# zhyever/PatchFusion

Hardware: NVIDIA H100
Metric: tiles/s (higher is better)
Workload: dtype bf16

## Files before the change

### patchfusion_b200/csrc/pf_api.cu

```cuda
#include <cuda_bf16.h>
#include <stdarg.h>
#include <stdio.h>
#include <stdlib.h>
#include <string.h>

#include <atomic>
#include <mutex>
#include <unordered_map>
#include <vector>

#include "pf_kernels.h"

namespace pf {

static thread_local char g_err[512] = "";
static std::atomic<long long> g_launches{0};

int set_error(const char* fmt, ...) {
  va_list ap;
  va_start(ap, fmt);
  vsnprintf(g_err, sizeof(g_err), fmt, ap);
  va_end(ap);
  return 1;
}
// ... 26 lines not shown
  }
}
static std::atomic<int> g_opt[6] = {{-1}, {-1}, {-1}, {-1}, {-1}, {-1}};
int option(int which) {
  static const char* names[6] = {"PF_OPT_TMA_EPILOGUE", "PF_OPT_HALO_MULTICAST", "PF_OPT_GEMM_MULTICAST", "PF_OPT_FUSED_RESAMPLE", "PF_OPT_PDL", "PF_OPT_RESIZE_SEPARABLE"};
  static const int defaults[6] = {1, 1, 1, 0, 0, 0};
  if (which < 0 || which > 5) return 0;
  int v = g_opt[which].load(std::memory_order_relaxed);
  if (v < 0) {
    const char* e = getenv(names[which]);
    if (!e && which == PF_OPT_PDL) e = getenv("PF_B200_PDL");
    v = e ? atoi(e) : defaults[which];
    g_opt[which].store(v, std::memory_order_relaxed);
  }
  return v;
}
bool pdl_enabled() {
  return option(PF_OPT_PDL) != 0;
}
int check_launch(const char* what) {
  cudaError_t e = cudaGetLastError();
  if (e != cudaSuccess) return set_error("%s launch: %s", what, cudaGetErrorString(e));
  count_launch(what);
  return 0;
}

typedef CUresult (*EncodeTiledFn)(CUtensorMap*, CUtensorMapDataType, cuuint32_t, void*, const cuuint64_t*,
                                  const cuuint64_t*, const cuuint32_t*, const cuuint32_t*, CUtensorMapInterleave,
                                  CUtensorMapSwizzle, CUtensorMapL2promotion, CUtensorMapFloatOOBfill);

static EncodeTiledFn encode_fn() {
  static EncodeTiledFn fn = nullptr;
  static std::once_flag once;
  std::call_once(once, [] {
    void* p = nullptr;
    cudaDriverEntryPointQueryResult q;
    if (cudaGetDriverEntryPoint("cuTensorMapEncodeTiled", &p, cudaEnableDefault, &q) == cudaSuccess &&
        q == cudaDriverEntryPointSuccess)
      fn = reinterpret_cast<EncodeTiledFn>(p);
  });
  return fn;
}

struct MapKey {
  uint64_t v[12];
  bool operator==(const MapKey& o) const { return memcmp(v, o.v, sizeof(v)) == 0; }
};
struct MapKeyHash {
  size_t operator()(const MapKey& k) const {
    uint64_t h = 1469598103934665603ull;
    for (int i = 0; i < 12; ++i) { h ^= k.v[i]; h *= 1099511628211ull; }
    return static_cast<size_t>(h);
  }
};
static std::unordered_map<MapKey, CUtensorMap, MapKeyHash> g_maps;
static std::mutex g_maps_mu;

static int encode(CUtensorMap* out, const void* ptr, int rank, const uint64_t* dims, const uint64_t* strides_bytes,
                  const uint32_t* box, CUtensorMapDataType dt = CU_TENSOR_MAP_DATA_TYPE_BFLOAT16) {
  MapKey key;
  memset(&key, 0, sizeof(key));
  key.v[0] = reinterpret_cast<uint64_t>(ptr);
  key.v[1] = static_cast<uint64_t>(rank) | (static_cast<uint64_t>(dt) << 8);
  for (int i = 0; i < rank; ++i) {
    key.v[2 + i] = dims[i];
    key.v[6 + i] = (i + 1 < rank ? strides_bytes[i] : 0) ^ (static_cast<uint64_t>(box[i]) << 48);
  }
  {
    std::lock_guard<std::mutex> g(g_maps_mu);
    auto it = g_maps.find(key);
    if (it != g_maps.end()) { *out = it->second; return 0; }
  }
  EncodeTiledFn fn = encode_fn();
  if (!fn) return set_error("cuTensorMapEncodeTiled entry point unavailable (no CUDA driver?)");
  if (reinterpret_cast<uintptr_t>(ptr) & 15) return set_error("tensor map: base pointer not 16-byte aligned");
  cuuint64_t gdim[5];
  cuuint64_t gstr[4];
  cuuint32_t bx[5], es[5];
  for (int i = 0; i < rank; ++i) { gdim[i] = dims[i]; bx[i] = box[i]; es[i] = 1; }
  for (int i = 0; i + 1 < rank; ++i) {
    gstr[i] = strides_bytes[i];
    if (gstr[i] & 15) return set_error("tensor map: stride %d (%llu B) not a multiple of 16", i, (unsigned long long)gstr[i]);
  }
  CUresult r = fn(out, dt, rank, const_cast<void*>(ptr), gdim, gstr, bx, es,
                  CU_TENSOR_MAP_INTERLEAVE_NONE, CU_TENSOR_MAP_SWIZZLE_128B, CU_TENSOR_MAP_L2_PROMOTION_L2_256B,
                  CU_TENSOR_MAP_FLOAT_OOB_FILL_NONE);
  if (r != CUDA_SUCCESS) {
    return set_error("cuTensorMapEncodeTiled failed (%d): rank %d dims %llu %llu %llu %llu box %u %u %u %u", (int)r, rank,
                     (unsigned long long)dims[0], (unsigned long long)(rank > 1 ? dims[1] : 0),
                     (unsigned long long)(rank > 2 ? dims[2] : 0), (unsigned long long)(rank > 3 ? dims[3] : 0), box[0],
                     rank > 1 ? box[1] : 0, rank > 2 ? box[2] : 0, rank > 3 ? box[3] : 0);
  }
  std::lock_guard<std::mutex> g(g_maps_mu);
  if (g_maps.size() > 65536) g_maps.clear();
  g_maps.emplace(key, *out);
  return 0;
}

int tmap_2d_bf16(CUtensorMap* out, const void* ptr, uint64_t cols, uint64_t rows, uint64_t ld, uint32_t box_cols,
                 uint32_t box_rows) {
  uint64_t dims[2] = {cols, rows};
  uint64_t str[1] = {ld * 2};
  uint32_t box[2] = {box_cols, box_rows};
  return encode(out, ptr, 2, dims, str, box);
}
int tmap_2d_f32(CUtensorMap* out, const void* ptr, uint64_t cols, uint64_t rows, uint64_t ld, uint32_t box_cols,
                uint32_t box_rows) {
  uint64_t dims[2] = {cols, rows};
  uint64_t str[1] = {ld * 4};
  uint32_t box[2] = {box_cols, box_rows};
  return encode(out, ptr, 2, dims, str, box, CU_TENSOR_MAP_DATA_TYPE_FLOAT32);
}
int tmap_3d_bf16(CUtensorMap* out, const void* ptr, uint64_t d0, uint64_t d1, uint64_t d2, uint64_t ld1, uint64_t ld2,
                 uint32_t b0, uint32_t b1, uint32_t b2) {
  uint64_t dims[3] = {d0, d1, d2};
  uint64_t str[2] = {ld1 * 2, ld2 * 2};
  uint32_t box[3] = {b0, b1, b2};
  return encode(out, ptr, 3, dims, str, box);
}
int tmap_4d_nhwc_bf16(CUtensorMap* out, const void* ptr, uint64_t C, uint64_t W, uint64_t H, uint64_t N, uint64_t ld,
                      uint32_t box_c, uint32_t box_w, uint32_t box_h) {
  uint64_t dims[4] = {C, W, H, N};
  uint64_t str[3] = {ld * 2, ld * 2 * W, ld * 2 * W * H};
  uint32_t box[4] = {box_c, box_w, box_h, 1};
  return encode(out, ptr, 4, dims, str, box);
}

__global__ void pack_weight_kernel(const float* __restrict__ w, int N, int N_pad, int num_src, int c0, int c1, int c2,
                                   int taps, const float* __restrict__ scale, __nv_bfloat16* __restrict__ dst,
                                   int Ktot) {
  long long idx = blockIdx.x * static_cast<long long>(blockDim.x) + threadIdx.x;
  long long total = static_cast<long long>(N_pad) * Ktot;
  if (idx >= total) return;
  int n = static_cast<int>(idx / Ktot);
  int k = static_cast<int>(idx - static_cast<long long>(n) * Ktot);
  int cs[3] = {c0, c1, c2};
  int ctot = c0 + (num_src > 1 ? c1 : 0) + (num_src > 2 ? c2 : 0);
  float v = 0.0f;
  int cbase = 0, kbase = 0;
  for (int s = 0; s < num_src; ++s) {
    int cp = (cs[s] + 63) / 64 * 64;
    int seg = taps * cp;
    if (k < kbase + seg) {
      int kk = k - kbase;
      int tap = kk / cp, c = kk - tap * cp;
      if (n < N && c < cs[s]) {
        v = w[(static_cast<long long>(n) * ctot + cbase + c) * taps + tap];
        if (scale) v *= scale[n];
      }
      break;
    }
    kbase += seg;
    cbase += cs[s];
  }
  dst[idx] = __float2bfloat16(v);
}

__global__ void pack_convT_kernel(const float* __restrict__ w, int Cin, int Cout, int k, __nv_bfloat16* __restrict__ dst,
                                  int Kp) {
  long long idx = blockIdx.x * static_cast<long long>(blockDim.x) + threadIdx.x;
  int Cp = (Cout + 31) / 32 * 32;
  long long total = static_cast<long long>(k) * k * Cp * Kp;
  if (idx >= total) return;
  int row = static_cast<int>(idx / Kp);
  int ci = static_cast<int>(idx - static_cast<long long>(row) * Kp);
  int tap = row / Cp, co = row - tap * Cp;
  float v = 0.0f;
  if (ci < Cin && co < Cout) v = w[(static_cast<long long>(ci) * Cout + co) * k * k + tap];
// ... 139 lines not shown
  } else if (u->a_mode == 1) {
    int bh = u->bh, bw = u->bw;
    if (bh == 0 || bw == 0) choose_tile(u->H, u->W, &bh, &bw);
    if (bh * bw != 128) return set_error("pf_gemm: bh*bw must be 128");
    d.bh = bh; d.bw = bw;
    d.tiles_y = (u->H + bh - 1) / bh; d.tiles_x = (u->W + bw - 1) / bw;
    d.m_tiles = u->NB * d.tiles_y * d.tiles_x;
    for (int s = 0; s < u->num_src; ++s)
      if (tmap_4d_nhwc_bf16(&tmA[s], u->a_ptr[s], u->a_c[s], u->W, u->H, u->NB, u->a_ld[s], 64, bw, bh)) return 1;
  } else {
    d.m_tiles = (u->M + 127) / 128;
    for (int s = 0; s < u->num_src; ++s)
      if (tmap_2d_bf16(&tmA[s], u->a_ptr[s], u->a_c[s], u->M, u->a_ld[s], 64, 128)) return 1;
  }
  u->bh = d.bh; u->bw = d.bw; u->tiles_y = d.tiles_y; u->tiles_x = d.tiles_x; u->m_tiles = d.m_tiles;
  int bn = u->block_n;
  if (bn == 0) {
    if (halo) {
      bn = n_pad % 192 == 0 ? 192 : (n_pad % 128 == 0 ? 128 : (n_pad % 64 == 0 ? 64 : 32));
    } else if (u->ps > 1 || u->w2) {
      const int span = u->ps > 1 ? (u->ps_cout + 31) / 32 * 32 : n_pad;
      for (int w : kGemmWidths)
        if (span % w == 0) bn = w;
      if (u->w2 && bn != n_pad) return set_error("pf_gemm: fused trailing layer needs the whole row in one N tile (N %d)", u->N);
    } else if (n_pad % 128 == 0) {
      const long long t128 = static_cast<long long>(d.m_tiles) * (n_pad / 128), sms = sm_count();
      const long long waves128 = (t128 + sms - 1) / sms, waves256 = (t128 / 2 + sms - 1) / sms;
      bn = n_pad % 256 == 0 && 2 * waves256 <= waves128 ? 256 : 128;
    } else {
      for (int w : kGemmWidths)
        if (n_pad % w == 0) bn = w;
    }
  }
  d.block_n = bn; d.N = u->N; d.n_tiles = (u->N + bn - 1) / bn;
  u->block_n = bn; u->n_tiles = d.n_tiles;
  if (tmap_2d_bf16(&tmB, u->w_ptr, u->Ktot, static_cast<uint64_t>(d.n_tiles) * bn, u->Ktot, 64, bn)) return 1;
  d.bias = u->bias; d.act = u->act;
  d.res1 = static_cast<const __nv_bfloat16*>(u->res1);
  d.res2 = static_cast<const __nv_bfloat16*>(u->res2);
  d.res_ld = u->res_ld;
  d.gamma = u->gamma;
  d.out = u->out; d.out_f32 = u->out_f32 || u->gamma != nullptr; d.out_ld = u->out_ld; d.out_col0 = u->out_col0;
  d.out2 = static_cast<__nv_bfloat16*>(u->out2); d.out2_ld = u->out2_ld;
  if ((u->out_f32 || u->gamma) && reinterpret_cast<uintptr_t>(u->out) % 32 != 0)
    return set_error("pf_gemm: fp32 outputs must be 32-byte aligned (256-bit epilogue stores)");
  d.wide = ((reinterpret_cast<uintptr_t>(u->out) | reinterpret_cast<uintptr_t>(u->out2) | reinterpret_cast<uintptr_t>(u->res1) |
             reinterpret_cast<uintptr_t>(u->res2)) % 32 == 0) &&
           u->out_col0 % 16 == 0 && (d.out_f32 || u->out_ld % 16 == 0) && (!u->out2 || u->out2_ld % 16 == 0) &&
           (!(u->res1 || u->res2) || u->res_ld % 16 == 0);
  d.ps = u->ps > 1 ? u->ps : 1;
  d.n_logical = u->N;
  if (d.ps > 1) {
    if (u->a_mode != 0) return set_error("pf_gemm: pixel shuffle needs a_mode 0");
    int cpad = (u->ps_cout + 31) / 32 * 32;
    if (cpad % bn != 0) return set_error("pf_gemm: padded ps_cout %d must be a multiple of block_n %d", cpad, bn);
    if (u->N != d.ps * d.ps * cpad) return set_error("pf_gemm: pixel shuffle N %d != k*k*pad32(Cout) %d", u->N, d.ps * d.ps * cpad);
    d.ps_cout_pad = cpad;
    d.n_logical = u->ps_cout;
  }
  d.w2 = u->w2; d.b2 = u->b2; d.n2 = u->n2; d.act2 = u->act2; d.skip_main = u->skip_main;
  d.out3 = u->out3; d.out3_ld = u->out3_ld;
  if (d.w2) {
    if (d.n_tiles != 1) return set_error("pf_gemm: fused trailing layer needs the whole row in one N tile (N %d)", u->N);
    if (d.n2 < 1 || d.n2 > 16 || !d.out3) return set_error("pf_gemm: fused trailing layer n2 %d (1..16), out3 required", d.n2);
    if (u->N % 4) return set_error("pf_gemm: fused trailing layer needs N % 4 == 0");
  }
  d.vt = static_cast<__nv_bfloat16*>(u->vt);
  d.vt_col0 = u->vt_col0; d.vt_seq = u->vt_seq; d.vt_seq_pad = u->vt_seq_pad; d.vt_dim = u->vt_dim;
  if (d.vt && (d.vt_col0 % bn) != 0) return set_error("pf_gemm: vt_col0 must be a multiple of block_n");
  int cl = 1;
  if (d.m_tiles >= 4 && static_cast<long long>(d.m_tiles) * d.n_tiles >= sm_count()) {
    if (halo) cl = option(PF_OPT_HALO_MULTICAST) >= 2 ? 4 : (option(PF_OPT_HALO_MULTICAST) == 1 ? 2 : 1);
    else if (option(PF_OPT_GEMM_MULTICAST) != 0 && u->a_mode == 0 && d.ps == 1 && bn % 16 == 0) cl = 2;
  }
  d.halo_cl = halo ? cl : 1;
  const bool mc = cl > 1;
  CUtensorMap tmBh;
  if (mc && tmap_2d_bf16(&tmBh, u->w_ptr, u->Ktot, static_cast<uint64_t>(d.n_tiles) * bn, u->Ktot, 64, bn / cl)) return 1;
  const bool no_tma_epi = option(PF_OPT_TMA_EPILOGUE) == 0;
  CUtensorMap tmOut;
  d.tma_out = 0;
  const uint64_t ocols = static_cast<uint64_t>(u->out_col0) + u->N;
  const bool ends16 = ocols % (d.out_f32 ? 4 : 8) == 0;
  if (!no_tma_epi && !halo && d.ps == 1 && !d.w2 && !d.res1 && !d.res2 && !d.out2 && ends16) {
    if (!d.out_f32 && bn % 64 == 0 && reinterpret_cast<uintptr_t>(u->out) % 16 == 0) {
      if (u->a_mode == 0) {
        if (tmap_2d_bf16(&tmOut, u->out, ocols, u->M, u->out_ld, 64, 16)) return 1;
      } else {
        const uint32_t bwx = d.bw < 16 ? d.bw : 16;
        if (tmap_4d_nhwc_bf16(&tmOut, u->out, ocols, u->W, u->H, u->NB, u->out_ld, 64, bwx, 16 / bwx)) return 1;
      }
      d.tma_out = 1;
    } else if (d.out_f32 && u->a_mode == 0 && u->out_ld % 4 == 0 && reinterpret_cast<uintptr_t>(u->out) % 16 == 0) {
      if (tmap_2d_f32(&tmOut, u->out, ocols, u->M, u->out_ld, 32, 16)) return 1;
      d.tma_out = 2;
    }
  }
  return gemm_launch(d, tmA, tmB, mc ? &tmBh : nullptr, d.tma_out ? &tmOut : nullptr, static_cast<cudaStream_t>(stream));
}

}
```

### patchfusion_b200/csrc/pf_gemm.cu

```cuda
#include "pf_common.cuh"
#include "pf_kernels.h"

namespace pf {

constexpr int kBlockM = 128;
constexpr int kBlockK = 64;
constexpr int kATileBytes = kBlockM * kBlockK * 2;
constexpr int kEpiWarps = 8;
constexpr int kGemmThreads = (kEpiWarps + 1) * 32;
constexpr int kHaloThreads = (kEpiWarps + 3) * 32;
constexpr int kRsWarp0 = kEpiWarps;
constexpr int kMaxSmem = 227 * 1024;
constexpr int kXposeWarp = 16 * 32 * 4;
constexpr int kStageWarp = 2 * kXposeWarp;
constexpr int kBarBytes = 512;

__host__ __device__ constexpr int gemm_stage_bytes(int bn) { return kATileBytes + bn * kBlockK * 2; }
__host__ __device__ constexpr int gemm_stages(int bn) {
  return (kMaxSmem - 1024  - kBarBytes - kEpiWarps * kStageWarp) / gemm_stage_bytes(bn) < 8
             ? (kMaxSmem - 1024 - kBarBytes - kEpiWarps * kStageWarp) / gemm_stage_bytes(bn)
             : 8;
}

struct GemmKernelParams {
// ... 254 lines not shown
__device__ __forceinline__ void epilogue_row(const GemmDesc& d, const float (&acc)[S], float* buf, int lane,
                                             const TileCoord& c, int ocol0, long long orow, bool row_ok,
                                             float (&y2)[kMaxTail]) {
  const int r = lane & 15;
  const float* rowp = buf + r * 32;
  const int sw = xpose16_swz(r) ^ (lane & 16);
  for (int k = 0; 32 * k < 2 * S && c.n0 + 32 * k < d.N; ++k) {
    acc_stage16_k(k, acc, buf, lane);
    __syncwarp();
    epilogue_cols<16, TAILN>(d, rowp, sw, 32 * k + (lane & 16), c, ocol0, orow, row_ok, y2);
    __syncwarp();
  }
}


struct EpiTma {
  const CUtensorMap* tm;
  uint32_t stg;
  uint8_t* stg_ptr;
  int cur;
};

__device__ __forceinline__ int epi_stage_acquire(EpiTma& e, int lane) {
  if (lane == 0) bulk_wait_read1();
  __syncwarp();
  const int off = e.cur * kXposeWarp;
  e.cur ^= 1;
  return off;
}

template <int S, int K = 0>
__device__ __forceinline__ void acc_chunk(int k, const float (&a)[S], float (&v)[16]) {
  if constexpr (K + 1 < S / 16) {
    if (k != K) { acc_chunk<S, K + 1>(k, a, v); return; }
  }
#pragma unroll
  for (int i = 0; i < 16; ++i) v[i] = a[16 * K + i];
}

__device__ __forceinline__ void epi_act(const GemmDesc& d, float (&f)[16]) {
  if (d.act == PF_ACT_RELU) {
#pragma unroll
    for (int j = 0; j < 16; ++j) f[j] = fmaxf(f[j], 0.0f);
  } else if (d.act == PF_ACT_GELU) {
#pragma unroll
    for (int j = 0; j < 16; j += 2) gelu_erf2(f[j], f[j + 1]);
  } else if (d.act == PF_ACT_SOFTPLUS) {
#pragma unroll
    for (int j = 0; j < 16; ++j) f[j] = softplus(f[j]);
  }
}
__device__ __forceinline__ float2 epi_vec2(const float* p, int col, int n_logical) {
  if (col + 1 < n_logical) return __ldg(reinterpret_cast<const float2*>(p + col));
  return make_float2(col < n_logical ? __ldg(p + col) : 0.f, 0.f);
}
__device__ __forceinline__ void epi_frag(const GemmDesc& d, float (&v)[16], int col, bool scale) {
  if (d.bias != nullptr) {
#pragma unroll
    for (int j = 0; j < 4; ++j) {
      const float2 b = epi_vec2(d.bias, col + 8 * j, d.n_logical);
      v[4 * j] += b.x; v[4 * j + 1] += b.y; v[4 * j + 2] += b.x; v[4 * j + 3] += b.y;
    }
  }
  epi_act(d, v);
  if (scale) {
#pragma unroll
    for (int j = 0; j < 4; ++j) {
      const float2 g = epi_vec2(d.gamma, col + 8 * j, d.n_logical);
      v[4 * j] *= g.x; v[4 * j + 1] *= g.y; v[4 * j + 2] *= g.x; v[4 * j + 3] *= g.y;
    }
  }
}

__device__ __forceinline__ void epi_tma_store(const GemmDesc& d, const EpiTma& e, const uint8_t* tile, const TileCoord& c,
                                              int warp, int col) {
  if (d.a_mode == 1) {
    const int r0 = warp * 16;
    const int yy = r0 / d.bw, xx = r0 - yy * d.bw;
    tma_store_4d(e.tm, tile, col, c.x0 + xx, c.y0 + yy, c.img);
  } else {
    tma_store_2d(e.tm, tile, col, c.m0 + warp * 16);
  }
}
template <int S>
__device__ __forceinline__ void epilogue_tile_tma_bf16(const GemmDesc& d, EpiTma& e, const float (&acc)[S],
                                                       const TileCoord& c, int warp, int lane) {
  const int oct = lane >> 4;
  const uint32_t lane_off = (lane & 15) * 128;
  for (int g = 0; 64 * g < 2 * S; ++g) {
    const int lcol = c.n0 + g * 64;
    if (lcol >= d.n_logical) break;
    const int tile = epi_stage_acquire(e, lane);
#pragma unroll
    for (int h = 0; h < 2; ++h) {
      float v[16];
      acc_chunk(2 * g + h, acc, v);
      epi_frag(d, v, lcol + 32 * h + 2 * (lane & 3), false);
#pragma unroll
      for (int p = 0; p < 2; ++p) {
        const int o = 4 * h + 2 * p;
        const uint32_t addr = e.stg + tile + lane_off + (((o + oct) ^ (lane & 7)) << 4);
        stmatrix_x4(addr, pack_bf16(v[8 * p], v[8 * p + 1]), pack_bf16(v[8 * p + 2], v[8 * p + 3]),
                        pack_bf16(v[8 * p + 4], v[8 * p + 5]), pack_bf16(v[8 * p + 6], v[8 * p + 7]));
      }
    }
    fence_proxy_async_smem();
    __syncwarp();
    if (lane == 0) {
      epi_tma_store(d, e, e.stg_ptr + tile, c, warp, d.out_col0 + lcol);
      bulk_commit();
    }
  }
}

template <int S>
__device__ __forceinline__ void epilogue_tile_tma_f32(const GemmDesc& d, EpiTma& e, const float (&acc)[S],
                                                      const TileCoord& c, int warp, int lane) {
  const int r = lane >> 2, q = lane & 3;
  const uint32_t lane_off = r * 128 + (q & 1) * 8;
  for (int ch = 0; 32 * ch < 2 * S; ++ch) {
    const int lcol = c.n0 + ch * 32;
    if (lcol >= d.n_logical) break;
    const int tile = epi_stage_acquire(e, lane);
    float v[16];
    acc_chunk(ch, acc, v);
    epi_frag(d, v, lcol + 2 * q, d.gamma != nullptr);
#pragma unroll
    for (int j = 0; j < 4; ++j) {
      const uint32_t addr = e.stg + tile + lane_off + (((2 * j + (q >> 1)) ^ r) << 4);
      st_shared_v2f(addr, v[4 * j], v[4 * j + 1]);
      st_shared_v2f(addr + 8 * 128, v[4 * j + 2], v[4 * j + 3]);
    }
    fence_proxy_async_smem();
    __syncwarp();
    if (lane == 0) {
      if (d.gamma != nullptr) tma_reduce_add_2d(e.tm, e.stg_ptr + tile, d.out_col0 + lcol, c.m0 + warp * 16);
      else tma_store_2d(e.tm, e.stg_ptr + tile, d.out_col0 + lcol, c.m0 + warp * 16);
      bulk_commit();
    }
  }
}

struct TileIter {
  int first, step, count, rank, n_tiles, cl;
  __device__ __forceinline__ int tile(int i) const {
    if (cl == 1) return i;
    const int nt = i % n_tiles, mp = i / n_tiles;
    return (cl * mp + rank) * n_tiles + nt;
  }
};
__device__ __forceinline__ TileIter make_iter(const GemmDesc& d, int total_tiles, int cl) {
  TileIter it;
  it.cl = cl; it.n_tiles = d.n_tiles;
  if (cl == 1) { it.first = blockIdx.x; it.step = gridDim.x; it.count = total_tiles; it.rank = 0; }
  else { it.first = blockIdx.x / cl; it.step = gridDim.x / cl; it.count = ((d.m_tiles + cl - 1) / cl) * d.n_tiles; it.rank = cluster_ctarank(); }
  return it;
}

__device__ __forceinline__ void tail_store(const GemmDesc& d, long long orow, const float (&y2)[kMaxTail]) {
  float* op = d.out3 + orow * d.out3_ld;
#pragma unroll
  for (int i = 0; i < kMaxTail; ++i) {
    if (i < d.n2) {
      float v2 = y2[i] + (d.b2 != nullptr ? __ldg(d.b2 + i) : 0.f);
      if (d.act2 == PF_ACT_RELU) v2 = fmaxf(v2, 0.f);
      else if (d.act2 == PF_ACT_SOFTPLUS) v2 = softplus(v2);
      else if (d.act2 == PF_ACT_GELU) v2 = gelu_erf(v2);
      op[i] = v2;
    }
  }
}

template <int S>
__device__ __forceinline__ void epilogue_tile(const GemmDesc& d, const TileCoord& c, const float (&acc)[S], int warp,
                                              int lane, float* buf, EpiTma* et) {
  const int r = 16 * warp + (lane & 15);
  bool row_ok;
  long long orow;
  if (d.a_mode == 1) {
    const int yy = r / d.bw, xx = r - yy * d.bw;
    const int y = c.y0 + yy, x = c.x0 + xx;
    row_ok = (y < d.H) && (x < d.W) && (c.img < d.NB);
    orow = (static_cast<long long>(c.img) * d.H + y) * d.W + x;
  } else {
    const int m = c.m0 + r;
    row_ok = m < d.M;
    orow = m;
  }
  int ocol0 = c.n0;
  if (d.ps > 1 && d.a_mode == 0) {
    const int tap = c.n0 / d.ps_cout_pad;
    ocol0 = c.n0 - tap * d.ps_cout_pad;
    const int ky = tap / d.ps, kx = tap - ky * d.ps;
    const int m = c.m0 + r;
    const int img = m / (d.H * d.W);
    const int rem = m - img * d.H * d.W;
    const int y = rem / d.W, x = rem - y * d.W;
    orow = (static_cast<long long>(img) * d.H * d.ps + y * d.ps + ky) * (d.W * d.ps) + x * d.ps + kx;
  }
  if (et != nullptr && d.tma_out != 0 && !(d.vt != nullptr && c.n0 >= d.vt_col0)) {
    if (d.tma_out == 2) {
      epilogue_tile_tma_f32(d, *et, acc, c, warp, lane);
    } else if constexpr (S % 32 == 0) {
      epilogue_tile_tma_bf16(d, *et, acc, c, warp, lane);
    }
    return;
  }
  if (et != nullptr && d.tma_out != 0) {
    if (lane == 0) bulk_wait_read0();
    __syncwarp();
  }
  float y2[kMaxTail];
#pragma unroll
  for (int i = 0; i < kMaxTail; ++i) y2[i] = 0.f;
  if (d.w2 == nullptr) epilogue_row<0>(d, acc, buf, lane, c, ocol0, orow, row_ok, y2);
  else if (d.n2 <= 1) epilogue_row<1>(d, acc, buf, lane, c, ocol0, orow, row_ok, y2);
  else if (d.n2 <= 4) epilogue_row<4>(d, acc, buf, lane, c, ocol0, orow, row_ok, y2);
  else epilogue_row<kMaxTail>(d, acc, buf, lane, c, ocol0, orow, row_ok, y2);
  if (d.w2 != nullptr) {
#pragma unroll
    for (int i = 0; i < kMaxTail; ++i)
      if (i < d.n2) y2[i] += __shfl_xor_sync(0xffffffffu, y2[i], 16);
    if (row_ok && lane < 16) tail_store(d, orow, y2);
  }
}

template <int CL>
__device__ __forceinline__ void release_stage(uint64_t* bar, int lane) {
  __syncwarp();
  if (lane == 0) {
    if (CL > 1) {
#pragma unroll
      for (int r = 0; r < CL; ++r) mbar_arrive_cluster(bar, r);
    } else {
      mbar_arrive(bar);
    }
  }
}

#ifdef PF_GEMM_TIMELINE
constexpr int kTimelineSlots = 8;
__device__ unsigned long long g_gemm_timeline[kTimelineSlots];
struct GemmTimeline {
  long long v[5] = {0, 0, 0, 0, 0};
  __device__ __forceinline__ long long now() const { return clock64(); }
  __device__ __forceinline__ void add(int i, long long t0) { v[i] += clock64() - t0; }
  __device__ __forceinline__ void tile() { v[0] += 1; }
  __device__ __forceinline__ void flush(int slot0, int n) const {
    for (int i = 0; i < n; ++i) atomicAdd(&g_gemm_timeline[slot0 + i], static_cast<unsigned long long>(v[i]));
  }
};
#else
struct GemmTimeline {
  __device__ __forceinline__ long long now() const { return 0; }
  __device__ __forceinline__ void add(int, long long) {}
  __device__ __forceinline__ void tile() {}
  __device__ __forceinline__ void flush(int, int) const {}
};
#endif

template <bool MC, int BN>
__global__ void __launch_bounds__(kGemmThreads, 1) pf_gemm_kernel(const __grid_constant__ GemmKernelParams P) {
  constexpr int CL = MC ? 2 : 1;
  constexpr int stage_bytes = gemm_stage_bytes(BN);
  constexpr int stages = gemm_stages(BN);
  extern __shared__ uint8_t smem_raw[];
  const GemmDesc& d = P.d;
  uint8_t* smem = reinterpret_cast<uint8_t*>((reinterpret_cast<uintptr_t>(smem_raw) + 1023) & ~uintptr_t(1023));
  uint8_t* xpose = smem + stages * stage_bytes;
  uint64_t* full_bar = reinterpret_cast<uint64_t*>(xpose + kEpiWarps * kStageWarp);
  uint64_t* empty_bar = full_bar + stages;

  const int warp = threadIdx.x >> 5;
  const int lane = threadIdx.x & 31;
  pdl_launch_dependents();

  constexpr int kTmaWarp = kEpiWarps;
  if (warp == kTmaWarp && lane == 0) {
    for (int s = 0; s < d.num_src; ++s) prefetch_tmap(&P.tmA[s]);
    prefetch_tmap(&P.tmB);
    for (int s = 0; s < stages; ++s) { mbar_init(&full_bar[s], 1); mbar_init(&empty_bar[s], kEpiWarps * CL); }
    if (d.tma_out) prefetch_tmap(&P.tmOut);
    fence_barrier_init();
  }
  __syncthreads();
  if (MC) cluster_sync_all();
  const TileIter it = make_iter(d, P.total_tiles, CL);
// ... 13 lines not shown
            int dy = d.taps == 9 ? tap / 3 - 1 : 0;
            int dx = d.taps == 9 ? tap % 3 - 1 : 0;
            for (int ch = 0; ch < d.chunks[s]; ++ch, ++kb) {
              const long long tl_w = tl.now();
              mbar_wait(&empty_bar[stage], phase ^ 1);
              tl.add(1, tl_w);
              uint8_t* sa = smem + stage * stage_bytes;
              uint8_t* sb = sa + kATileBytes;
              if (elect_one()) {
                mbar_expect_tx(&full_bar[stage], stage_bytes);
                if (d.a_mode == 0) tma_load_2d(sa, &P.tmA[s], &full_bar[stage], ch * kBlockK, c.m0);
                else tma_load_4d(sa, &P.tmA[s], &full_bar[stage], ch * kBlockK, c.x0 + dx, c.y0 + dy, c.img);
                if (MC) {
                  constexpr int half_rows = BN / 2;
                  tma_load_2d_mc(sb + it.rank * half_rows * 128, &P.tmBh, &full_bar[stage], kb * kBlockK,
                                 c.n0 + it.rank * half_rows, static_cast<uint16_t>(3));
                } else {
                  tma_load_2d(sb, &P.tmB, &full_bar[stage], kb * kBlockK, c.n0);
                }
              }
              if (++stage == stages) { stage = 0; phase ^= 1; }
            }
          }
        }
      }
      tl.add(2, tl_start);
      if (lane == 0) tl.flush(0, 3);
    }
  } else {
    EpiTma et;
    et.tm = &P.tmOut; et.stg_ptr = xpose + warp * kStageWarp; et.stg = smem_u32(et.stg_ptr); et.cur = 0;
    float* buf = reinterpret_cast<float*>(et.stg_ptr);
    const uint32_t a_off = static_cast<uint32_t>((warp >> 2) * 64 * 128);
    float acc[BN / 2];
    int stage = 0; uint32_t phase = 0;
    int rs = 0;
    GemmTimeline tl;
    const long long tl_start = tl.now();
    for (int ti = it.first; ti < it.count; ti += it.step) {
      const TileCoord c = decode_tile(d, it.tile(ti));
      tl.tile();
      const long long tl_main = tl.now();
      uint32_t accum = 0;
      for (int kb = 0; kb < P.k_steps; ++kb) {
        const long long tl_w = tl.now();
        mbar_wait(&full_bar[stage], phase);
        tl.add(1, tl_w);
        const uint32_t sa = smem_u32(smem + stage * stage_bytes);
        const uint64_t adesc = wgmma_desc_k128(sa + a_off);
        const uint64_t bdesc = wgmma_desc_k128(sa + kATileBytes);
        wgmma_fence();
#pragma unroll
        for (int k = 0; k < kBlockK / 16; ++k) Wgmma<BN>::ss(acc, adesc + 2 * k, bdesc + 2 * k, accum | k);
        wgmma_commit();
        accum = 1;
        wgmma_wait<1>();
        if (kb > 0) {
          release_stage<CL>(&empty_bar[rs], lane);
          if (++rs == stages) rs = 0;
        }
        if (++stage == stages) { stage = 0; phase ^= 1; }
      }
      wgmma_wait<0>();
      release_stage<CL>(&empty_bar[rs], lane);
      if (++rs == stages) rs = 0;
      tl.add(2, tl_main);
      const long long tl_epi = tl.now();
      epilogue_tile(d, c, acc, warp, lane, buf, &et);
      __syncwarp();
      tl.add(3, tl_epi);
    }
    if (lane == 0) bulk_wait0();
    tl.add(4, tl_start);
    if (lane == 0 && (warp & 3) == 0) tl.flush(3, 5);
  }
  __syncthreads();
  if (MC) cluster_sync_all();
}

constexpr int kHaloW = 10, kHaloH = 18;
constexpr int kHaloBytes = kHaloW * kHaloH * 128;
constexpr int kHaloSlot = 24 * 1024;
constexpr int kHaloSlots = 3;
constexpr int kHaloBBytes = kMaxSmem - 1024  - kBarBytes - kEpiWarps * kXposeWarp - kHaloSlots * kHaloSlot;
__host__ __device__ constexpr int halo_kc(int bn) {
  return 2 * 9 * bn * kBlockK * 2 <= kHaloBBytes ? 9 : (2 * 3 * bn * kBlockK * 2 <= kHaloBBytes ? 3 : 1);
}
__host__ __device__ constexpr int halo_stages(int bn) {
  return kHaloBBytes / (halo_kc(bn) * bn * kBlockK * 2) < 6 ? kHaloBBytes / (halo_kc(bn) * bn * kBlockK * 2) : 6;
}


__device__ __forceinline__ void rs_coord(int dst, int in, float scale, int& lo, int& hi, float& frac) {
  const float src = scale * dst;
  lo = static_cast<int>(src);
  if (lo > in - 1) lo = in - 1;
  hi = lo + (lo < in - 1 ? 1 : 0);
  frac = src - lo;
}
__device__ __forceinline__ void halo_fill_bilinear(uint32_t slot, const GemmDesc& d, int s, int ch, const TileCoord& c, int lane) {
  const int ih = d.rs_h[s], iw = d.rs_w[s], ld = d.rs_ld[s];
  const __nv_bfloat16* src = d.rs_ptr[s] + static_cast<size_t>(c.img) * ih * iw * ld + ch * kBlockK;
  const int cvalid = d.k_true[s] - ch * kBlockK;
  const float sy = d.rs_sy[s], sx = d.rs_sx[s];
  const int j = lane & 7;
  const bool jok = j * 8 < cvalid && c.img < d.NB;
#pragma unroll 5
  for (int p = lane >> 3; p < kHaloW * kHaloH; p += 4) {
    const int hy = p / kHaloW, hx = p - hy * kHaloW;
    const int Y = c.y0 - 1 + hy, X = c.x0 - 1 + hx;
    uint32_t o0 = 0, o1 = 0, o2 = 0, o3 = 0;
    if (jok && Y >= 0 && Y < d.H && X >= 0 && X < d.W) {
      int y0, y1, x0, x1; float fy, fx;
      rs_coord(Y, ih, sy, y0, y1, fy);
      rs_coord(X, iw, sx, x0, x1, fx);
      const __nv_bfloat16* r0 = src + static_cast<size_t>(y0) * iw * ld + j * 8;
      const __nv_bfloat16* r1 = src + static_cast<size_t>(y1) * iw * ld + j * 8;
      const uint4 ua = __ldg(reinterpret_cast<const uint4*>(r0 + static_cast<size_t>(x0) * ld));
      const uint4 ub = __ldg(reinterpret_cast<const uint4*>(r0 + static_cast<size_t>(x1) * ld));
      const uint4 uc = __ldg(reinterpret_cast<const uint4*>(r1 + static_cast<size_t>(x0) * ld));
      const uint4 ud = __ldg(reinterpret_cast<const uint4*>(r1 + static_cast<size_t>(x1) * ld));
      const float w00 = (1.f - fy) * (1.f - fx), w01 = (1.f - fy) * fx, w10 = fy * (1.f - fx), w11 = fy * fx;
      const uint64_t p00 = pack2f(w00, w00), p01 = pack2f(w01, w01), p10 = pack2f(w10, w10), p11 = pack2f(w11, w11);
      const uint32_t wa[4] = {ua.x, ua.y, ua.z, ua.w}, wb[4] = {ub.x, ub.y, ub.z, ub.w};
      const uint32_t wc[4] = {uc.x, uc.y, uc.z, uc.w}, wd[4] = {ud.x, ud.y, ud.z, ud.w};
      uint32_t ow[4];
#pragma unroll
      for (int k = 0; k < 4; ++k) {
        uint64_t r = mul2(p00, pack2(wa[k] << 16, wa[k] & 0xffff0000u));
        r = fma2(p01, pack2(wb[k] << 16, wb[k] & 0xffff0000u), r);
        r = fma2(p10, pack2(wc[k] << 16, wc[k] & 0xffff0000u), r);
        r = fma2(p11, pack2(wd[k] << 16, wd[k] & 0xffff0000u), r);
        float lo, hi;
        unpack2f(r, lo, hi);
        ow[k] = pack_bf16(lo, hi);
      }
      o0 = ow[0]; o1 = ow[1]; o2 = ow[2]; o3 = ow[3];
    }
    st_shared_v4(slot + p * 128 + ((j ^ (p & 7)) << 4), o0, o1, o2, o3);
  }
}

__device__ __forceinline__ void halo_a_frags(uint32_t ra, int lane, uint32_t (&fa)[4][4]) {
  const uint32_t sw = (ra >> 7) & 7;
#pragma unroll
  for (int k = 0; k < kBlockK / 16; ++k) ldmatrix_x4(ra + (((2 * k + (lane >> 4)) ^ sw) << 4), fa[k]);
}

template <int CL, int BN>
__global__ void __launch_bounds__(kHaloThreads, 1) pf_conv3_halo_kernel(const __grid_constant__ GemmKernelParams P) {
  constexpr bool MC = CL > 1;
  constexpr uint16_t kMask = static_cast<uint16_t>((1u << CL) - 1);
  constexpr int kc = halo_kc(BN);
  constexpr int b_tile_bytes = BN * kBlockK * 2;
  constexpr int b_stage_bytes = kc * b_tile_bytes;
  constexpr int stages = halo_stages(BN);
  extern __shared__ uint8_t smem_raw[];
  const GemmDesc& d = P.d;
  uint8_t* smem = reinterpret_cast<uint8_t*>((reinterpret_cast<uintptr_t>(smem_raw) + 1023) & ~uintptr_t(1023));
  uint8_t* smem_b = smem + kHaloSlots * kHaloSlot;
  uint8_t* xpose = smem_b + stages * b_stage_bytes;
  uint64_t* bars = reinterpret_cast<uint64_t*>(xpose + kEpiWarps * kXposeWarp);
  uint64_t* a_full = bars;
  uint64_t* a_empty = a_full + kHaloSlots;
  uint64_t* b_full = a_empty + kHaloSlots;
  uint64_t* b_empty = b_full + stages;

  const int warp = threadIdx.x >> 5;
  const int lane = threadIdx.x & 31;
  pdl_launch_dependents();
  constexpr int kTmaWarp = kRsWarp0 + 2;
  if (warp == kTmaWarp && lane == 0) {
    for (int s = 0; s < d.num_src; ++s) if (d.rs_h[s] == 0) prefetch_tmap(&P.tmA[s]);
    prefetch_tmap(&P.tmB);
    for (int s = 0; s < kHaloSlots; ++s) { mbar_init(&a_full[s], 1); mbar_init(&a_empty[s], kEpiWarps); }
    for (int s = 0; s < stages; ++s) { mbar_init(&b_full[s], 1); mbar_init(&b_empty[s], kEpiWarps * CL); }
    fence_barrier_init();
  }
  __syncthreads();
  if (MC) cluster_sync_all();
  const TileIter it = make_iter(d, P.total_tiles, CL);
  pdl_wait();

  if (warp >= kEpiWarps) {
    if (warp == kTmaWarp) {
      int as = 0; uint32_t aph = 0;
      int bs = 0; uint32_t bph = 0;
      for (int ti = it.first; ti < it.count; ti += it.step) {
        TileCoord c = decode_tile(d, it.tile(ti));
        int kbase = 0;
        for (int s = 0; s < d.num_src; ++s) {
          const int nch = d.chunks[s];
          for (int ch = 0; ch < nch; ++ch) {
            if (d.rs_h[s] == 0) {
              mbar_wait(&a_empty[as], aph ^ 1);
              if (elect_one()) {
                mbar_expect_tx(&a_full[as], kHaloBytes);
                tma_load_4d(smem + as * kHaloSlot, &P.tmA[s], &a_full[as], ch * kBlockK, c.x0 - 1, c.y0 - 1, c.img);
              }
            }
            if (++as == kHaloSlots) { as = 0; aph ^= 1; }
            for (int tap0 = 0; tap0 < 9; tap0 += kc) {
              mbar_wait(&b_empty[bs], bph ^ 1);
              if (elect_one()) {
                mbar_expect_tx(&b_full[bs], b_stage_bytes);
                if (MC) {
                  constexpr int part_rows = BN / CL;
                  for (int j = 0; j < kc; ++j)
                    tma_load_2d_mc(smem_b + bs * b_stage_bytes + j * b_tile_bytes + it.rank * part_rows * 128, &P.tmBh,
                                   &b_full[bs], (kbase + (tap0 + j) * nch + ch) * kBlockK, c.n0 + it.rank * part_rows,
                                   kMask);
                } else {
                  for (int j = 0; j < kc; ++j)
                    tma_load_2d(smem_b + bs * b_stage_bytes + j * b_tile_bytes, &P.tmB, &b_full[bs],
                                (kbase + (tap0 + j) * nch + ch) * kBlockK, c.n0);
                }
              }
              if (++bs == stages) { bs = 0; bph ^= 1; }
            }
          }
          kbase += 9 * nch;
        }
      }
    } else if (warp < kRsWarp0 + 2 && d.rs_any) {
      int as = 0; uint32_t aph = 0;
      int turn = 0;
      for (int ti = it.first; ti < it.count; ti += it.step) {
        TileCoord c = decode_tile(d, it.tile(ti));
        for (int s = 0; s < d.num_src; ++s) {
          for (int ch = 0; ch < d.chunks[s]; ++ch) {
            if (d.rs_h[s] != 0) {
              if ((turn & 1) == warp - kRsWarp0) {
                mbar_wait(&a_empty[as], aph ^ 1);
                halo_fill_bilinear(smem_u32(smem + as * kHaloSlot), d, s, ch, c, lane);
                __syncwarp();
                if (lane == 0) mbar_arrive(&a_full[as]);
              }
              ++turn;
            }
            if (++as == kHaloSlots) { as = 0; aph ^= 1; }
          }
        }
      }
    }
  } else {
    float* buf = reinterpret_cast<float*>(xpose + warp * kXposeWarp);
    const int arow = 16 * warp + (lane & 15);
    const uint32_t a_off = static_cast<uint32_t>(((arow >> 3) * kHaloW + (arow & 7)) * 128);
    float acc[BN / 2];
    uint32_t fa[2][4][4];
    int as = 0; uint32_t aph = 0;
    int bs = 0; uint32_t bph = 0;
    int rbs = 0;
    for (int ti = it.first; ti < it.count; ti += it.step) {
      const TileCoord c = decode_tile(d, it.tile(ti));
      uint32_t accum = 0;
      for (int s = 0; s < d.num_src; ++s) {
        for (int ch = 0; ch < d.chunks[s]; ++ch) {
          mbar_wait(&a_full[as], aph);
          const uint32_t a_base = smem_u32(smem + as * kHaloSlot) + a_off;
          uint32_t sb = 0;
#pragma unroll
          for (int tap = 0; tap < 9; ++tap) {
            if (tap % kc == 0) {
              mbar_wait(&b_full[bs], bph);
              sb = smem_u32(smem_b + bs * b_stage_bytes);
              if (++bs == stages) { bs = 0; bph ^= 1; }
            }
            halo_a_frags(a_base + static_cast<uint32_t>(((tap / 3) * kHaloW + tap % 3) * 128), lane, fa[tap & 1]);
            const uint64_t bdesc = wgmma_desc_k128(sb + (tap % kc) * b_tile_bytes);
            wgmma_fence();
#pragma unroll
            for (int k = 0; k < kBlockK / 16; ++k) Wgmma<BN>::rs(acc, fa[tap & 1][k], bdesc + 2 * k, accum | k);
            wgmma_commit();
            accum = 1;
            wgmma_wait<1>();
            if (tap > 0 && tap % kc == 0) {
              release_stage<CL>(&b_empty[rbs], lane);
              if (++rbs == stages) rbs = 0;
            }
          }
          wgmma_wait<0>();
          release_stage<CL>(&b_empty[rbs], lane);
          if (++rbs == stages) rbs = 0;
          release_stage<1>(&a_empty[as], lane);
          if (++as == kHaloSlots) { as = 0; aph ^= 1; }
        }
      }
      epilogue_tile(d, c, acc, warp, lane, buf, nullptr);
      __syncwarp();
    }
  }
  __syncthreads();
  if (MC) cluster_sync_all();
}


static int g_sm_counts[kMaxDevices] = {0};

using KernelFn = void (*)(GemmKernelParams);
template <int CL>
static KernelFn halo_kernel_cl(int bn) {
  switch (bn) {
    case 32: return pf_conv3_halo_kernel<CL, 32>;
    case 64: return pf_conv3_halo_kernel<CL, 64>;
    case 128: return pf_conv3_halo_kernel<CL, 128>;
    case 192: return pf_conv3_halo_kernel<CL, 192>;
    default: return nullptr;
  }
}
static KernelFn halo_kernel(int cl, int bn) {
  return cl == 4 ? halo_kernel_cl<4>(bn) : (cl == 2 ? halo_kernel_cl<2>(bn) : halo_kernel_cl<1>(bn));
}
template <bool MC>
static KernelFn gemm_kernel_mc(int bn) {
  switch (bn) {
    case 32: return pf_gemm_kernel<MC, 32>;
    case 64: return pf_gemm_kernel<MC, 64>;
    case 96: return pf_gemm_kernel<MC, 96>;
    case 128: return pf_gemm_kernel<MC, 128>;
    case 192: return pf_gemm_kernel<MC, 192>;
    case 256: return pf_gemm_kernel<MC, 256>;
    default: return nullptr;
  }
}
static KernelFn gemm_kernel(bool mc, int bn) { return mc ? gemm_kernel_mc<true>(bn) : gemm_kernel_mc<false>(bn); }

int gemm_launch(const GemmDesc& d, const CUtensorMap* tmA, const CUtensorMap& tmB, const CUtensorMap* tmBh,
                const CUtensorMap* tmOut, cudaStream_t stream) {
  static bool attr_done[kMaxDevices] = {false};
  const int dev = current_device();
  if (!attr_done[dev]) {
    cudaError_t e = cudaSuccess;
    for (bool mc : {false, true})
      for (int bn : kGemmWidths)
        if (e == cudaSuccess) e = cudaFuncSetAttribute(gemm_kernel(mc, bn), cudaFuncAttributeMaxDynamicSharedMemorySize, kMaxSmem);
    for (int cl : {1, 2, 4})
      for (int bn : {32, 64, 128, 192})
        if (e == cudaSuccess) e = cudaFuncSetAttribute(halo_kernel(cl, bn), cudaFuncAttributeMaxDynamicSharedMemorySize, kMaxSmem);
    if (e != cudaSuccess) return set_error("cudaFuncSetAttribute(gemm kernels): %s", cudaGetErrorString(e));
    cudaDeviceGetAttribute(&g_sm_counts[dev], cudaDevAttrMultiProcessorCount, dev);
    attr_done[dev] = true;
  }
  const int g_sm_count = g_sm_counts[dev];
  {
    const long long rows = d.a_mode == 1 ? static_cast<long long>(d.NB) * d.H * d.W : d.M;
    int ktrue = 0;
    for (int s = 0; s < d.num_src; ++s) ktrue += d.k_true[s];
    const int n_true = d.ps > 1 ? d.n_logical * d.ps * d.ps : d.N;
    note_work(2.0 * rows * ktrue * d.taps * n_true, "%s rows%lld K%dx%d N%d%s%s%s", d.taps == 9 ? "conv3x3" : (d.a_mode == 1 ? "conv1x1" : (d.ps > 1 ? "convT" : "linear")),
              rows, d.taps, ktrue, n_true, d.act ? (d.act == PF_ACT_GELU ? " gelu" : (d.act == PF_ACT_RELU ? " relu" : " softplus")) : "",
              d.gamma ? " gamma" : (d.vt ? " vt" : ""), d.w2 ? " tail" : "");
  }
  GemmKernelParams P;
  for (int s = 0; s < d.num_src; ++s) P.tmA[s] = tmA[s];
  for (int s = d.num_src; s < 3; ++s) P.tmA[s] = tmA[0];
  P.tmB = tmB;
  P.tmBh = tmBh ? *tmBh : tmB;
  P.tmOut = tmOut ? *tmOut : tmB;
  P.d = d;
  if (d.tma_out && !tmOut) return set_error("gemm: tma_out without an output tensor map");
  int ks = 0;
  for (int s = 0; s < d.num_src; ++s) ks += d.chunks[s] * d.taps;
  P.k_steps = ks;
  P.total_tiles = d.m_tiles * d.n_tiles;
  if (P.total_tiles <= 0 || ks <= 0) return set_error("gemm: empty problem");
  int grid = P.total_tiles < g_sm_count ? P.total_tiles : g_sm_count;
  if (d.halo) {
    const KernelFn hk = halo_kernel(d.halo_cl, d.block_n);
    if (hk == nullptr) return set_error("conv3 halo: block_n %d (32, 64, 128 or 192)", d.block_n);
    const int b_bytes = halo_kc(d.block_n) * d.block_n * kBlockK * 2;
    const int hstages = halo_stages(d.block_n);
    size_t hsmem = 1024 + static_cast<size_t>(kHaloSlots) * kHaloSlot + static_cast<size_t>(hstages) * b_bytes +
                   kEpiWarps * kXposeWarp + kBarBytes;
    cudaError_t le;
    if (tmBh != nullptr) {
      const int cl = d.halo_cl;
      const int groups = ((d.m_tiles + cl - 1) / cl) * d.n_tiles;
      cudaLaunchConfig_t cfg = {};
      cfg.blockDim = dim3(kHaloThreads); cfg.dynamicSmemBytes = hsmem; cfg.stream = stream;
      cudaLaunchAttribute at[2];
      at[0].id = cudaLaunchAttributeClusterDimension;
      at[0].val.clusterDim.x = cl; at[0].val.clusterDim.y = 1; at[0].val.clusterDim.z = 1;
      at[1].id = cudaLaunchAttributeProgrammaticStreamSerialization;
      at[1].val.programmaticStreamSerializationAllowed = 1;
      cfg.attrs = at;
      cfg.numAttrs = 1;
      static int max_clusters[kMaxDevices][5] = {};
      if (max_clusters[dev][cl] == 0) {
        cfg.gridDim = dim3(cl * (g_sm_count / cl));
        int n = 0;
        cudaError_t qe = cudaOccupancyMaxActiveClusters(&n, hk, &cfg);
        if (qe != cudaSuccess || n < 1) { cudaGetLastError(); n = g_sm_count / cl; }
        max_clusters[dev][cl] = n < g_sm_count / cl ? n : g_sm_count / cl;
      }
      const int clusters = groups < max_clusters[dev][cl] ? groups : max_clusters[dev][cl];
      cfg.gridDim = dim3(cl * clusters);
      cfg.numAttrs = pdl_enabled() ? 2 : 1;
      le = cudaLaunchKernelEx(&cfg, hk, P);
    } else {
      le = launch_pdl(hk, dim3(grid), dim3(kHaloThreads), hsmem, stream, P);
    }
    if (le != cudaSuccess) return set_error("pf_conv3_halo_kernel launch: %s", cudaGetErrorString(le));
  } else {
    const KernelFn gk = gemm_kernel(tmBh != nullptr, d.block_n);
    if (gk == nullptr) return set_error("gemm: block_n %d (32, 64, 96, 128, 192 or 256)", d.block_n);
    const size_t smem = 1024 + static_cast<size_t>(gemm_stages(d.block_n)) * gemm_stage_bytes(d.block_n) +
                        kEpiWarps * kStageWarp + kBarBytes;
    cudaError_t le;
    if (tmBh != nullptr) {
      const int pairs = ((d.m_tiles + 1) / 2) * d.n_tiles;
      const int clusters = pairs < g_sm_count / 2 ? pairs : g_sm_count / 2;
      cudaLaunchConfig_t cfg = {};
      cfg.gridDim = dim3(2 * clusters); cfg.blockDim = dim3(kGemmThreads); cfg.dynamicSmemBytes = smem; cfg.stream = stream;
      cudaLaunchAttribute at[2];
      at[0].id = cudaLaunchAttributeClusterDimension;
      at[0].val.clusterDim.x = 2; at[0].val.clusterDim.y = 1; at[0].val.clusterDim.z = 1;
      at[1].id = cudaLaunchAttributeProgrammaticStreamSerialization;
      at[1].val.programmaticStreamSerializationAllowed = 1;
      cfg.attrs = at;
      cfg.numAttrs = pdl_enabled() ? 2 : 1;
      le = cudaLaunchKernelEx(&cfg, gk, P);
    } else {
      le = launch_pdl(gk, dim3(grid), dim3(kGemmThreads), smem, stream, P);
    }
    if (le != cudaSuccess) return set_error("pf_gemm_kernel launch: %s", cudaGetErrorString(le));
  }
  cudaError_t e = cudaGetLastError();
  if (e != cudaSuccess) return set_error("pf_gemm_kernel launch: %s", cudaGetErrorString(e));
  count_launch(d.halo ? "pf_conv3_halo_kernel" : "pf_gemm_kernel");
  return 0;
}


}

extern "C" int pf_gemm_timeline(unsigned long long* out, int32_t reset) {
#ifdef PF_GEMM_TIMELINE
  static_assert(pf::kTimelineSlots == PF_GEMM_TIMELINE_SLOTS, "timeline slots");
  cudaError_t e = cudaDeviceSynchronize();
  if (e == cudaSuccess && out != nullptr)
    e = cudaMemcpyFromSymbol(out, pf::g_gemm_timeline, sizeof(unsigned long long) * pf::kTimelineSlots);
  if (e == cudaSuccess && reset) {
    const unsigned long long zero[pf::kTimelineSlots] = {};
    e = cudaMemcpyToSymbol(pf::g_gemm_timeline, zero, sizeof(zero));
  }
  if (e != cudaSuccess) return pf::set_error("pf_gemm_timeline: %s", cudaGetErrorString(e));
  return 0;
#else
  (void)out; (void)reset;
  return pf::set_error("pf_gemm_timeline: library built without -DPF_GEMM_TIMELINE");
#endif
}
```

Measured before the change: 104.1.

## Enable TMA-store epilogue for conv3 halo kernel with 32-column swizzled groups

Extends the TMA bulk-store epilogue to the 3x3 halo conv kernel, which previously always used the scalar/transpose epilogue. Adds 32-wide group support with 64B swizzle for block_n 32, and doubles per-warp staging smem for halo, which shrinks the weight ring. It also adds timeline instrumentation in the producer and consumer loops. The aim is to overlap output stores with compute and cut epilogue store cost, at the price of fewer B stages and some timing overhead.

```diff
diff --git a/patchfusion_b200/csrc/pf_api.cu b/patchfusion_b200/csrc/pf_api.cu
--- a/patchfusion_b200/csrc/pf_api.cu
+++ b/patchfusion_b200/csrc/pf_api.cu
@@ -132,8 +132,10 @@
     gstr[i] = strides_bytes[i];
     if (gstr[i] & 15) return set_error("tensor map: stride %d (%llu B) not a multiple of 16", i, (unsigned long long)gstr[i]);
   }
+  const uint32_t row_bytes = box[0] * (dt == CU_TENSOR_MAP_DATA_TYPE_FLOAT32 ? 4 : 2);
+  const CUtensorMapSwizzle swz = row_bytes == 64 ? CU_TENSOR_MAP_SWIZZLE_64B : CU_TENSOR_MAP_SWIZZLE_128B;
   CUresult r = fn(out, dt, rank, const_cast<void*>(ptr), gdim, gstr, bx, es,
-                  CU_TENSOR_MAP_INTERLEAVE_NONE, CU_TENSOR_MAP_SWIZZLE_128B, CU_TENSOR_MAP_L2_PROMOTION_L2_256B,
+                  CU_TENSOR_MAP_INTERLEAVE_NONE, swz, CU_TENSOR_MAP_L2_PROMOTION_L2_256B,
                   CU_TENSOR_MAP_FLOAT_OOB_FILL_NONE);
   if (r != CUDA_SUCCESS) {
     return set_error("cuTensorMapEncodeTiled failed (%d): rank %d dims %llu %llu %llu %llu box %u %u %u %u", (int)r, rank,
@@ -439,16 +441,17 @@
   d.tma_out = 0;
   const uint64_t ocols = static_cast<uint64_t>(u->out_col0) + u->N;
   const bool ends16 = ocols % (d.out_f32 ? 4 : 8) == 0;
-  if (!no_tma_epi && !halo && d.ps == 1 && !d.w2 && !d.res1 && !d.res2 && !d.out2 && ends16) {
-    if (!d.out_f32 && bn % 64 == 0 && reinterpret_cast<uintptr_t>(u->out) % 16 == 0) {
+  if (!no_tma_epi && !(halo && any_rs) && d.ps == 1 && !d.w2 && !d.res1 && !d.res2 && !d.out2 && ends16) {
+    const uint32_t group = halo && bn == 32 ? 32 : 64;
+    if (!d.out_f32 && bn % group == 0 && reinterpret_cast<uintptr_t>(u->out) % 16 == 0) {
       if (u->a_mode == 0) {
         if (tmap_2d_bf16(&tmOut, u->out, ocols, u->M, u->out_ld, 64, 16)) return 1;
       } else {
         const uint32_t bwx = d.bw < 16 ? d.bw : 16;
-        if (tmap_4d_nhwc_bf16(&tmOut, u->out, ocols, u->W, u->H, u->NB, u->out_ld, 64, bwx, 16 / bwx)) return 1;
+        if (tmap_4d_nhwc_bf16(&tmOut, u->out, ocols, u->W, u->H, u->NB, u->out_ld, group, bwx, 16 / bwx)) return 1;
       }
       d.tma_out = 1;
-    } else if (d.out_f32 && u->a_mode == 0 && u->out_ld % 4 == 0 && reinterpret_cast<uintptr_t>(u->out) % 16 == 0) {
+    } else if (d.out_f32 && u->a_mode == 0 &&u->out_ld % 4 == 0 && reinterpret_cast<uintptr_t>(u->out) % 16 == 0) {
       if (tmap_2d_f32(&tmOut, u->out, ocols, u->M, u->out_ld, 32, 16)) return 1;
       d.tma_out = 2;
     }
diff --git a/patchfusion_b200/csrc/pf_gemm.cu b/patchfusion_b200/csrc/pf_gemm.cu
--- a/patchfusion_b200/csrc/pf_gemm.cu
+++ b/patchfusion_b200/csrc/pf_gemm.cu
@@ -360,24 +360,26 @@
     tma_store_2d(e.tm, tile, col, c.m0 + warp * 16);
   }
 }
-template <int S>
+template <int G, int S>
 __device__ __forceinline__ void epilogue_tile_tma_bf16(const GemmDesc& d, EpiTma& e, const float (&acc)[S],
                                                        const TileCoord& c, int warp, int lane) {
+  static_assert(G == 64 || G == 32, "group width");
   const int oct = lane >> 4;
-  const uint32_t lane_off = (lane & 15) * 128;
-  for (int g = 0; 64 * g < 2 * S; ++g) {
-    const int lcol = c.n0 + g * 64;
+  const uint32_t lane_off = (lane & 15) * (2 * G);
+  const int swz = G == 64 ? (lane & 7) : ((lane >> 1) & 3);
+  for (int g = 0; G * g < 2 * S; ++g) {
+    const int lcol = c.n0 + g * G;
     if (lcol >= d.n_logical) break;
     const int tile = epi_stage_acquire(e, lane);
 #pragma unroll
-    for (int h = 0; h < 2; ++h) {
+    for (int h = 0; h < G / 32; ++h) {
       float v[16];
-      acc_chunk(2 * g + h, acc, v);
+      acc_chunk(G / 32 * g + h, acc, v);
       epi_frag(d, v, lcol + 32 * h + 2 * (lane & 3), false);
 #pragma unroll
       for (int p = 0; p < 2; ++p) {
         const int o = 4 * h + 2 * p;
-        const uint32_t addr = e.stg + tile + lane_off + (((o + oct) ^ (lane & 7)) << 4);
+        const uint32_t addr = e.stg + tile + lane_off + (((o + oct) ^ swz) << 4);
         stmatrix_x4(addr, pack_bf16(v[8 * p], v[8 * p + 1]), pack_bf16(v[8 * p + 2], v[8 * p + 3]),
                         pack_bf16(v[8 * p + 4], v[8 * p + 5]), pack_bf16(v[8 * p + 6], v[8 * p + 7]));
       }
@@ -480,7 +482,7 @@
     if (d.tma_out == 2) {
       epilogue_tile_tma_f32(d, *et, acc, c, warp, lane);
     } else if constexpr (S % 32 == 0) {
-      epilogue_tile_tma_bf16(d, *et, acc, c, warp, lane);
+      epilogue_tile_tma_bf16<64>(d, *et, acc, c, warp, lane);
     }
     return;
   }
@@ -660,13 +662,16 @@
 constexpr int kHaloBytes = kHaloW * kHaloH * 128;
 constexpr int kHaloSlot = 24 * 1024;
 constexpr int kHaloSlots = 3;
-constexpr int kHaloBBytes = kMaxSmem - 1024  - kBarBytes - kEpiWarps * kXposeWarp - kHaloSlots * kHaloSlot;
+constexpr int kHaloBBytes = kMaxSmem - 1024  - kBarBytes - kEpiWarps * kStageWarp - kHaloSlots * kHaloSlot;
 __host__ __device__ constexpr int halo_kc(int bn) {
   return 2 * 9 * bn * kBlockK * 2 <= kHaloBBytes ? 9 : (2 * 3 * bn * kBlockK * 2 <= kHaloBBytes ? 3 : 1);
 }
 __host__ __device__ constexpr int halo_stages(int bn) {
   return kHaloBBytes / (halo_kc(bn) * bn * kBlockK * 2) < 6 ? kHaloBBytes / (halo_kc(bn) * bn * kBlockK * 2) : 6;
 }
+static_assert(halo_kc(32) == 9 && halo_stages(32) == 3 && halo_kc(64) == 3 && halo_stages(64) == 5 &&
+                  halo_kc(128) == 3 && halo_stages(128) == 2 && halo_kc(192) == 1 && halo_stages(192) == 5,
+              "halo weight ring");
 
 
 __device__ __forceinline__ void rs_coord(int dst, int in, float scale, int& lo, int& hi, float& frac) {
@@ -738,7 +743,7 @@
   uint8_t* smem = reinterpret_cast<uint8_t*>((reinterpret_cast<uintptr_t>(smem_raw) + 1023) & ~uintptr_t(1023));
   uint8_t* smem_b = smem + kHaloSlots * kHaloSlot;
   uint8_t* xpose = smem_b + stages * b_stage_bytes;
-  uint64_t* bars = reinterpret_cast<uint64_t*>(xpose + kEpiWarps * kXposeWarp);
+  uint64_t* bars = reinterpret_cast<uint64_t*>(xpose + kEpiWarps * kStageWarp);
   uint64_t* a_full = bars;
   uint64_t* a_empty = a_full + kHaloSlots;
   uint64_t* b_full = a_empty + kHaloSlots;
@@ -753,6 +758,7 @@
     prefetch_tmap(&P.tmB);
     for (int s = 0; s < kHaloSlots; ++s) { mbar_init(&a_full[s], 1); mbar_init(&a_empty[s], kEpiWarps); }
     for (int s = 0; s < stages; ++s) { mbar_init(&b_full[s], 1); mbar_init(&b_empty[s], kEpiWarps * CL); }
+    if (d.tma_out) prefetch_tmap(&P.tmOut);
     fence_barrier_init();
   }
   __syncthreads();
@@ -762,16 +768,21 @@
 
   if (warp >= kEpiWarps) {
     if (warp == kTmaWarp) {
+      GemmTimeline tl;
+      const long long tl_start = tl.now();
       int as = 0; uint32_t aph = 0;
       int bs = 0; uint32_t bph = 0;
       for (int ti = it.first; ti < it.count; ti += it.step) {
         TileCoord c = decode_tile(d, it.tile(ti));
+        tl.tile();
         int kbase = 0;
         for (int s = 0; s < d.num_src; ++s) {
           const int nch = d.chunks[s];
           for (int ch = 0; ch < nch; ++ch) {
             if (d.rs_h[s] == 0) {
+              const long long tl_w = tl.now();
               mbar_wait(&a_empty[as], aph ^ 1);
+              tl.add(1, tl_w);
               if (elect_one()) {
                 mbar_expect_tx(&a_full[as], kHaloBytes);
                 tma_load_4d(smem + as * kHaloSlot, &P.tmA[s], &a_full[as], ch * kBlockK, c.x0 - 1, c.y0 - 1, c.img);
@@ -779,7 +790,9 @@
             }
             if (++as == kHaloSlots) { as = 0; aph ^= 1; }
             for (int tap0 = 0; tap0 < 9; tap0 += kc) {
+              const long long tl_w = tl.now();
               mbar_wait(&b_empty[bs], bph ^ 1);
+              tl.add(1, tl_w);
               if (elect_one()) {
                 mbar_expect_tx(&b_full[bs], b_stage_bytes);
                 if (MC) {
@@ -800,6 +813,8 @@
           kbase += 9 * nch;
         }
       }
+      tl.add(2, tl_start);
+      if (lane == 0) tl.flush(0, 3);
     } else if (warp < kRsWarp0 + 2 && d.rs_any) {
       int as = 0; uint32_t aph = 0;
       int turn = 0;
@@ -822,7 +837,9 @@
       }
     }
   } else {
-    float* buf = reinterpret_cast<float*>(xpose + warp * kXposeWarp);
+    EpiTma et;
+    et.tm = &P.tmOut; et.stg_ptr = xpose + warp * kStageWarp; et.stg = smem_u32(et.stg_ptr); et.cur = 0;
+    float* buf = reinterpret_cast<float*>(et.stg_ptr);
     const int arow = 16 * warp + (lane & 15);
     const uint32_t a_off = static_cast<uint32_t>(((arow >> 3) * kHaloW + (arow & 7)) * 128);
     float acc[BN / 2];
@@ -830,18 +847,26 @@
     int as = 0; uint32_t aph = 0;
     int bs = 0; uint32_t bph = 0;
     int rbs = 0;
+    GemmTimeline tl;
+    const long long tl_start = tl.now();
     for (int ti = it.first; ti < it.count; ti += it.step) {
       const TileCoord c = decode_tile(d, it.tile(ti));
+      tl.tile();
+      const long long tl_main = tl.now();
       uint32_t accum = 0;
       for (int s = 0; s < d.num_src; ++s) {
         for (int ch = 0; ch < d.chunks[s]; ++ch) {
+          long long tl_w = tl.now();
           mbar_wait(&a_full[as], aph);
+          tl.add(1, tl_w);
           const uint32_t a_base = smem_u32(smem + as * kHaloSlot) + a_off;
           uint32_t sb = 0;
 #pragma unroll
           for (int tap = 0; tap < 9; ++tap) {
             if (tap % kc == 0) {
+              tl_w = tl.now();
               mbar_wait(&b_full[bs], bph);
+              tl.add(1, tl_w);
               sb = smem_u32(smem_b + bs * b_stage_bytes);
               if (++bs == stages) { bs = 0; bph ^= 1; }
             }
@@ -865,9 +890,16 @@
           if (++as == kHaloSlots) { as = 0; aph ^= 1; }
         }
       }
-      epilogue_tile(d, c, acc, warp, lane, buf, nullptr);
+      tl.add(2, tl_main);
+      const long long tl_epi = tl.now();
+      if (d.tma_out) epilogue_tile_tma_bf16<BN == 32 ? 32 : 64>(d, et, acc, c, warp, lane);
+      else epilogue_tile(d, c, acc, warp, lane, buf, nullptr);
       __syncwarp();
-    }
+      tl.add(3, tl_epi);
+    }
+    if (lane == 0) bulk_wait0();
+    tl.add(4, tl_start);
+    if (lane == 0 && (warp & 3) == 0) tl.flush(3, 5);
   }
   __syncthreads();
   if (MC) cluster_sync_all();
@@ -950,7 +982,7 @@
     const int b_bytes = halo_kc(d.block_n) * d.block_n * kBlockK * 2;
     const int hstages = halo_stages(d.block_n);
     size_t hsmem = 1024 + static_cast<size_t>(kHaloSlots) * kHaloSlot + static_cast<size_t>(hstages) * b_bytes +
-                   kEpiWarps * kXposeWarp + kBarBytes;
+                   kEpiWarps * kStageWarp + kBarBytes;
     cudaError_t le;
     if (tmBh != nullptr) {
       const int cl = d.halo_cl;
```

Result: faster. 111.5, median of 6 (+7.1%).
